# neobotix/neo_mpc_planner2

Hardware: AMD Instinct MI355X
Metric: MPC solves/sec (control_steps=3, 500x500 costmap) (higher is better)
Workload: dtype f64

## Files before the change

### neo_mpc_planner2_amd/csrc/costmap.h

```cpp
#pragma once
#include <hip/hip_runtime.h>
#include <math.h>
#include <stdint.h>

#include "neo_mpc_device.h"
#include "wave_ops.h"
#include "solver_context.h"
#include "fast_math.h"
#include "solver_rules.h"

namespace neo_mpc {
namespace {

__device__ __forceinline__ int cell_of(double w, double origin, double res, double inv) {
  double t = w - origin;
  double q = t * inv;
  double fl = floor(q);
  if (fabs(q - rint(q)) < 1e-6) fl = floor(t / res);
  int cell;
  asm("v_cvt_i32_f64 %0, %1" : "=v"(cell) : "v"(fl));
  return cell;
}

__device__ __forceinline__ int map_raw(const DevMap& m, int mx, int my) {
  if (mx < -m.border || my < -m.border || mx >= m.size_x + m.border || my >= m.size_y + m.border)
    return 254;
  return m.cells[(long)my * m.pitch + mx];
}

__device__ __forceinline__ int raw_occupancy(int raw) {
  return raw == 0 ? 0 : raw == 253 ? 99 : raw == 254 ? 100 : raw == 255 ? -1 : 1 + (97 * (raw - 1)) / 251;
}
__device__ __forceinline__ double raw_cost(int raw) { return (double)raw_occupancy(raw) / 100.0; }

template <bool kCovered = false>
__device__ __forceinline__ int cell_raw(const SolveArgs& a, const Ctx& c, const double* L, int mx, int my) {
  const unsigned tx = (unsigned)(mx - c.tile_x0), ty = (unsigned)(my - c.tile_y0);
  const int lg = c.tile_geom & 31;
  if (kCovered || ((tx >> lg) == 0u && ty < (unsigned)(c.tile_geom >> 8)))
    return reinterpret_cast<const uint8_t*>(L + a.lds.tile)[(ty << lg) + tx];
  return map_raw(a.map, mx, my);
}

template <bool kCovered = false>
__device__ __forceinline__ int step_raw(const SolveArgs& a, const Ctx& c, const double* L, double x, double y) {
  if (c.tile_geom & kTileFree) return 0;
  const double X = c.X0 + (c.c0 * x - c.s0 * y), Y = c.Y0 + (c.s0 * x + c.c0 * y);
  const int mx = cell_of(X, a.map.origin_x, a.map.resolution, a.map.inv_resolution);
  const int my = cell_of(Y, a.map.origin_y, a.map.resolution, a.map.inv_resolution);
  return cell_raw<kCovered>(a, c, L, mx, my);
}
template <bool kCovered = false>
__device__ __forceinline__ double step_term(const SolveArgs& a, const Ctx& c, const double* L, double x, double y) {
  return L[a.lds.term + step_raw<kCovered>(a, c, L, x, y)];
}

constexpr double kSticky = NEO_RULE_STICKY, kWall = NEO_RULE_WALL, kStickyDist = NEO_RULE_STICKY_DIST, kWallDist = NEO_RULE_WALL_DIST;
constexpr double kHopMargin = NEO_RULE_HOP_MARGIN;
template <bool kCovered = false>
__device__ __forceinline__ int edge_stickiness(const SolveArgs& a, const Ctx& c, const double* L, double x, double y,
                                               double cs, double sn, double& wxx, double& wxy, double& wyy, double& lx,
                                               double& ly, bool& hop, float& hop_x, float& hop_y) {
  wxx = 0.0; wxy = 0.0; wyy = 0.0; lx = 0.0; ly = 0.0;
  hop = false; hop_x = 0.0f; hop_y = 0.0f;
  if (c.tile_geom & kTileFree) return 0;
  const double X = c.X0 + (c.c0 * x - c.s0 * y), Y = c.Y0 + (c.s0 * x + c.c0 * y);
  const int mx = cell_of(X, a.map.origin_x, a.map.resolution, a.map.inv_resolution);
  const int my = cell_of(Y, a.map.origin_y, a.map.resolution, a.map.inv_resolution);
  const double fx = (X - a.map.origin_x) * a.map.inv_resolution - (double)mx;
  const double fy = (Y - a.map.origin_y) * a.map.inv_resolution - (double)my;
  const int raw_here = cell_raw<kCovered>(a, c, L, mx, my);
  const double here = L[a.lds.term + raw_here];
  const bool far = mx <= -2147483647 || mx >= 2147483646 || my <= -2147483647 || my >= 2147483646;
  if (far) return raw_here;
  const double hop_range = L[a.lds.tol + T_HOP_RANGE];
  const double zone = fmax(kWallDist, hop_range);
  const bool xlo = fx < zone, xhi = 1.0 - fx < zone, ylo = fy < zone, yhi = 1.0 - fy < zone;
  double rx = 0.0, ry = 0.0, pbx = 0.0, pby = 0.0;
  double drop = L[a.lds.tol + T_HOP_DROP], hwx = 0.0, hwy = 0.0;
  if (xlo || xhi) {
    const int raw_n = cell_raw<kCovered>(a, c, L, xlo ? mx - 1 : mx + 1, my);
    const double dist = xlo ? fx : 1.0 - fx, there = L[a.lds.term + raw_n];
    const bool wall = raw_n == 254 && raw_here != 254;
    if (wall) { if (dist < kWallDist) { rx = kWall * 2.0 * a.p.wt_n; pbx = (xlo ? kWallDist - dist : dist - kWallDist) * a.map.resolution; } }
    else if (dist < kStickyDist && there > here) rx = kSticky * 2.0 * a.p.wt_n;
    if (dist < hop_range && here - there > drop) {
      drop = here - there; hop = true;
      hwx = (xlo ? -1.0 : 1.0) * (dist + kHopMargin) * a.map.resolution; hwy = 0.0;
    }
  }
  if (ylo || yhi) {
    const int raw_n = cell_raw<kCovered>(a, c, L, mx, ylo ? my - 1 : my + 1);
    const double dist = ylo ? fy : 1.0 - fy, there = L[a.lds.term + raw_n];
    const bool wall = raw_n == 254 && raw_here != 254;
    if (wall) { if (dist < kWallDist) { ry = kWall * 2.0 * a.p.wt_n; pby = (ylo ? kWallDist - dist : dist - kWallDist) * a.map.resolution; } }
    else if (dist < kStickyDist && there > here) ry = kSticky * 2.0 * a.p.wt_n;
    if (dist < hop_range && here - there > drop) {
      hop = true;
      hwx = 0.0; hwy = (ylo ? -1.0 : 1.0) * (dist + kHopMargin) * a.map.resolution;
    }
  }
  wxx = rx * c.c0 * c.c0 + ry * c.s0 * c.s0;
  wxy = rx * c.c0 * -c.s0 + ry * c.s0 * c.c0;
  wyy = rx * c.s0 * c.s0 + ry * c.c0 * c.c0;
  lx = -(rx * pbx * c.c0 + ry * pby * c.s0);
  ly = -(rx * pbx * -c.s0 + ry * pby * c.c0);
  if (hop) {
    const double hrx = c.c0 * hwx + c.s0 * hwy, hry = -c.s0 * hwx + c.c0 * hwy, idt = rcp_fast(a.p.dt);
    hop_x = (float)((cs * hrx + sn * hry) * idt); hop_y = (float)((-sn * hrx + cs * hry) * idt);
  }
  return raw_here;
}

__device__ double edge_cost(const DevMap& m, double ax, double ay, double bx, double by) {
  int x0 = cell_of(ax, m.origin_x, m.resolution, m.inv_resolution);
  int y0 = cell_of(ay, m.origin_y, m.resolution, m.inv_resolution);
  const int x1 = cell_of(bx, m.origin_x, m.resolution, m.inv_resolution);
  const int y1 = cell_of(by, m.origin_y, m.resolution, m.inv_resolution);
  if (x0 < 0 || y0 < 0 || x0 >= m.size_x || y0 >= m.size_y || x1 < 0 || y1 < 0 || x1 >= m.size_x || y1 >= m.size_y)
    return raw_cost(254);
  const long dx = labs((long)x1 - x0), dy = labs((long)y1 - y0);
  const int sx = x1 >= x0 ? 1 : -1, sy = y1 >= y0 ? 1 : -1;
  long err = dx - dy;
  double worst = -1.0;
  for (long guard = 0; guard <= dx + dy + 1; ++guard) {
    worst = fmax(worst, raw_cost(map_raw(m, x0, y0)));
    if (x0 == x1 && y0 == y1) break;
    long e2 = 2 * err;
    if (e2 > -dy) { err -= dy; x0 += sx; }
    if (e2 < dx) { err += dx; y0 += sy; }
  }
  return worst;
}

__device__ double footprint_cost(const SolveArgs& a, const double* L, uint32_t b, int lane) {
  if (!a.footprints || a.footprint_points == 0) return L[a.lds.prob + P_FOOTPRINT];
  const int np = (int)a.footprint_points;
  const double* pts = a.footprints + (size_t)b * 2 * np;
  double worst = -1.0;
  for (int e = lane; e < np; e += kLanes) {
    int j = (e + 1) % np;
    worst = fmax(worst, edge_cost(a.map, pts[2 * e], pts[2 * e + 1], pts[2 * j], pts[2 * j + 1]));
  }
  return wave_max(worst);
}

}
}
```

### neo_mpc_planner2_amd/csrc/k1_solve.h

```cpp
#pragma once
#include <hip/hip_runtime.h>
#include <hip/hip_ext.h>
#include <math.h>
#include <stdint.h>
#include <stdlib.h>

#include "neo_mpc_device.h"
#include "wave_ops.h"
#include "fast_math.h"
#include "solver_context.h"
#include "solver_rules.h"
#include "costmap.h"
#include "feasible_set.h"
#include "rollout.h"
#include "riccati.h"
#include "adjoint.h"
#include "tangent_cone.h"
#include "dense_newton.h"
#include "lbfgs.h"
#include "cell_scan.h"
#include "k1_timing.h"

namespace neo_mpc {
namespace {
// ... 80 lines not shown
    load_records(a, L, b, lane);
    if (uniform_int(reinterpret_cast<const int*>(L + a.lds.prob)[PI_SKIP]) == 1) { skip_instance(a, b, lane); return false; }
    select_map(a.map, L + a.lds.prob);
    flags = reset_and_warm(a, L, b, lane) ? NEO_MPC_FLAG_RESET : 0;
    const double fcost = footprint_cost(a, L, b, lane);
    if (lane == 0) L[a.lds.prob + P_FOOTPRINT] = fcost;
    Ctx c;
    make_ctx_wave(p, a.map, L + a.lds.prob, fcost, c, lane);
    load_tile(a, c, L, lane);
    s.wall_in_reach = (c.tile_geom & kTileWall) != 0;
    if (s.wall_in_reach) flags |= NEO_MPC_FLAG_WALL_IN_REACH;
    if (lane == 0) {
      double* t = L + a.lds.tol;
      t[T_XTOL] = p.xtol; t[T_EARLY] = p.early_tol; t[T_FINAL] = p.final_tol; t[T_FTOL] = p.ftol;
      t[T_STALL] = p.stall_step; t[T_WTOL] = p.wtol; t[T_WTOL_LATE] = p.wtol_late; t[T_KINK] = p.kink_radius;
      t[T_KONST] = c.konst; t[T_TRUE_YAW] = c.true_yaw;
      t[T_HOP_DROP] = p.hop_min_drop; t[T_HOP_RANGE] = p.hop_range;
      t[T_BTOL_MAP] = p.btol_map; t[T_BTOL_FREE] = p.btol_free;
      reinterpret_cast<int*>(t + T_HOP_STAGE)[kHopLanes] = 0;
      t[T_C0] = c.c0; t[T_S0] = c.s0; t[T_TYAW] = c.tyaw; t[T_FYAW] = c.fyaw;
      int* ti = reinterpret_cast<int*>(t + T_TILE);
      ti[0] = c.tile_x0; ti[1] = c.tile_y0; ti[2] = c.tile_geom;
    }
    double* u = L + a.lds.u;
    for (int i = lane; i < n; i += kLanes) project_block<kTame>(p, u[3 * i], u[3 * i + 1], u[3 * i + 2]);
    WAVE_SYNC();
    for (int k = 0; k < nv; ++k) cold = cold && (u[k] == 0.0);
    ctx_from_lds<false>(a, L, c);
    {
      double* S = L + a.lds.state;
      int* Si = reinterpret_cast<int*>(S);
      const bool has_prev = uniform_int(Si[SI_HAS_PREV]) == 1 && !(flags & NEO_MPC_FLAG_RESET);
      WAVE_SYNC();
      if (lane == 0) {
        double q0 = has_prev ? S[S_PREV_U0] : u[nv - 3], q1 = has_prev ? S[S_PREV_U0 + 1] : u[nv - 2], q2 = has_prev ? S[S_PREV_U0 + 2] : u[nv - 1];
        project_block<kTame>(p, q0, q1, q2);
        S[S_PREV_U0] = q0; S[S_PREV_U0 + 1] = q1; S[S_PREV_U0 + 2] = q2;
        Si[SI_HAS_PREV] = 0;
      }
      WAVE_SYNC();
    }
    if (!cold && n > 1 && !(p.compat & kCompatNoUnshift) && p.max_it < kDumpGradient) {
      const double* A0 = L + a.lds.state + S_PREV_U0;
      double ts = 0.0;
      const double fs = rollout_cost<kSteps, kTame, kCovered>(
          a, c, L,
          [&](int i, double& b0, double& b1, double& b2) {
            const double* src = lane == 1 ? (i == 0 ? A0 : u + 3 * (i - 1)) : u + 3 * i;
            b0 = src[0]; b1 = src[1]; b2 = src[2];
          },
          NoRecord(), &ts);
      const double f_warm = lane_value(fs, 0), f_alt = lane_value(fs, 1);
      const bool free_both = lane_value(ts, 0) == 0.0 && lane_value(ts, 1) == 0.0;
      if (f_alt < f_warm && free_both) {
        double v0 = 0.0, v1 = 0.0, v2 = 0.0;
        const int k0 = lane, k1 = lane + kLanes, k2 = lane + 2 * kLanes;
        if (k0 < nv) v0 = k0 >= 3 ? u[k0 - 3] : A0[k0];
        if (k1 < nv) v1 = u[k1 - 3];
        if (k2 < nv) v2 = u[k2 - 3];
        WAVE_SYNC();
        if (k0 < nv) u[k0] = v0;
        if (k1 < nv) u[k1] = v1;
        if (k2 < nv) u[k2] = v2;
      } else if (f_alt < f_warm && lane == 0) {
        reinterpret_cast<int*>(L + a.lds.state)[SI_HAS_PREV] = kAltArmed;
      }
      WAVE_SYNC();
    }
  }
  s.flags = flags; s.cold = cold;
  return true;
}

template <int kMinWavesPerSimd, int kSteps, int kDir, bool kTame, int kStaticTile, int kLayoutSteps, bool kRouted = false>
__device__ __forceinline__ bool solve_search(double* L, uint32_t b, SolveCarry& sc) {
  constexpr bool kCovered = kStaticTile > 0;
  constexpr bool kNewton = kDir == 1;
  constexpr bool kRiccati = kDir == 2;
  constexpr bool kSecond = kDir != 0;
  constexpr bool kBlockedRule = kNewton || kRouted;
  static_assert(!kRiccati || kSteps == 0 || kRouted, "the stage-wise direction: run-time-sized, or the routed kernel's control_steps-3 branch");
  static_assert(!kRouted || (kRiccati && kSteps == kRoutedSteps), "the routed branch is the stage-wise one, three stages in registers");
  constexpr int kFew = (kRiccati && kSteps > 0) ? kSteps : 0;
  constexpr int kNwSteps = !kNewton ? 1 : kSteps ? kSteps : kNewtonMaxSteps;
  constexpr bool kVectorPose = kTame;
  constexpr int kRegSteps = kSteps ? kSteps : 1;
  constexpr int kPairs = kSteps ? 4 : NEO_MPC_MAX_LBFGS_MEMORY;
  double f = sc.f;
  const bool cold = sc.cold;
  int npairs = 0, head = 0, nfev = sc.nfev, it = sc.it, status = sc.status, stall = 0;
  int blocked_run = 0;
  int nblocked = 1;
  double u_term = 0.0;
  double gain1 = INFINITY, gain2 = INFINITY;
  bool final_step = false;
  double alpha = 1.0;
  bool scanned = false;
  int nscans = 0;
  bool scan_only = false;
  auto lane_again = []() {
    int zero;
    asm volatile("v_mov_b32 %0, 0" : "=v"(zero));
    return (int)__builtin_amdgcn_mbcnt_hi(~0u, __builtin_amdgcn_mbcnt_lo(~0u, (unsigned)zero));
  };
  NEO_SEGMENT_DECL;
  NEO_SEGMENT(0);
  for (;;) {
  SolveArgs a;
  fresh_args<kSteps, kStaticTile, kLayoutSteps, kRouted>(a);
  own_loop_params(a);
  select_map(a.map, L + a.lds.prob);
  const DevParams& p = a.p;
  const int n = kSteps ? kSteps : p.n, nv = 3 * n, mem = p.mem;
  double cand[3 * kRegSteps], cand_sn[kRegSteps], cand_cs[kRegSteps];
  bool have_trig = false;
  Ctx c;
  ctx_from_lds<kVectorPose>(a, L, c);
  double* u = L + a.lds.u;
  double* gs = L + a.lds.gs;
  double* gt = L + a.lds.gt;
  double* gr = L + a.lds.gr;
  double* d = L + a.lds.d;
  double* u_prev = L + a.lds.u_prev;
  double* gt_prev = L + a.lds.gt_prev;
  double* u_new = L + a.lds.u_new;
  double* ACS = L + a.lds.cs;
  double* ASN = L + a.lds.sn;
  int* AMODE = reinterpret_cast<int*>(L + a.lds.mode);
  static_assert(2 * 7 >= kNewtonRecord, "Newton records do not fit the step arrays");

  if (!scanned && nscans == 0) {
    const int lane = lane_again();
    for (int i = lane; i < n; i += kLanes) { AMODE[4 * i + 2] = 0; AMODE[4 * i + 3] = 0; }
    if (kRouted && lane == 0) L[a.lds.tol + T_KINK] = p.kink_radius_stagewise;
    alpha = kRiccati ? fmax(1.0, n * 0.125) : 1.0;
    if (kFew && lane == 0) { double* t = L + a.lds.tol; t[T_GAIN1] = INFINITY; t[T_GAIN2] = INFINITY; t[T_ALPHA] = alpha; }
    if (kRiccati && lane == 0) L[a.lds.tol + T_MU] = n > 8 ? (double)(n - 8) * 0.125 : 0.0;
  }
  bool v_feasible = false;
  if (kRiccati) {
    double b0 = c.v0, b1 = c.v1, b2 = c.v2;
    asm volatile("" : "+v"(b0), "+v"(b1), "+v"(b2));
    project_block<kTame>(p, b0, b1, b2);
    v_feasible = b0 == c.v0 && b1 == c.v1 && b2 == c.v2;
  }
  double my_scale;
  {
    int l0 = lane_again();
    my_scale = kRiccati ? 0.0 : lane_scale<kSecond>(l0);
  }
  for (; it < p.max_it && !scan_only; ++it) {
    int lane = lane_again();
    const bool exact_step = kRiccati && nblocked == 0;
    int tol_off = a.lds.tol;
    asm volatile("" : "+s"(tol_off));
    const double* TOL = L + tol_off;
    NEO_PHASE_DECL;
    NEO_PHASE(0);
    constexpr int kVars = 3 * kNwSteps;
    const int nvr = kSteps ? kVars : nv;
    bool free_path = false;
    int nhops = 0;
    float hc[kVars];
    float newton_sol = 0.0f;
    if (kNewton) {
      double hcol[kSteps ? kVars : 1];
      const double hstep = 1e-6, inv_h = 1.0 / hstep;
      double pcs[kNwSteps], psn[kNwSteps];
      double x = 0.0, y = 0.0, th = 0.0;
    #pragma unroll
      for (int i = 0; i < kNwSteps; ++i) {
        if (kSteps || i < n) {
          const double vx = u[3 * i] + (lane == 3 * i ? hstep : 0.0);
          const double vy = u[3 * i + 1] + (lane == 3 * i + 1 ? hstep : 0.0);
          const double w = u[3 * i + 2] + (lane == 3 * i + 2 ? hstep : 0.0);
          th += w * p.dt;
          sincos_heading<kTame>(th, &psn[i], &pcs[i]);
          x += (vx * pcs[i] - vy * psn[i]) * p.dt;
          y += (vx * psn[i] + vy * pcs[i]) * p.dt;
        }
      }
      double SX = 0.0, SY = 0.0, ST = 0.0;
    #pragma unroll
      for (int k = kNwSteps - 1; k >= 0; --k) {
        if (kSteps || k < n) {
          const double vx = u[3 * k] + (lane == 3 * k ? hstep : 0.0);
          const double vy = u[3 * k + 1] + (lane == 3 * k + 1 ? hstep : 0.0);
          const double w = u[3 * k + 2] + (lane == 3 * k + 2 ? hstep : 0.0);
          const double pdx = (vx * pcs[k] - vy * psn[k]) * p.dt, pdy = (vx * psn[k] + vy * pcs[k]) * p.dt;
          double prt = -2.0 * p.wo_n * (c.tyaw - th);
          if (k == n - 1) prt += -2.0 * p.wterm_o * (c.fyaw - th);
          SX += -2.0 * p.wt_n * (c.cx - x); SY += -2.0 * p.wt_n * (c.cy - y);
          ST += prt - pdy * SX + pdx * SY;
          const double g0 = p.dt * (pcs[k] * SX + psn[k] * SY), g1 = p.dt * (-psn[k] * SX + pcs[k] * SY),
                       g2 = p.dt * ST;
          if (kSteps) {
            hcol[3 * k] = g0; hcol[3 * k + 1] = g1; hcol[3 * k + 2] = g2;
          } else {
            const double b0 = lane_value(g0, 63), b1 = lane_value(g1, 63), b2 = lane_value(g2, 63);
            if (lane == 63) { gs[3 * k] = b0; gs[3 * k + 1] = b1; gs[3 * k + 2] = b2; }
            hc[3 * k] = (float)((g0 - b0) * inv_h);
            hc[3 * k + 1] = (float)((g1 - b1) * inv_h);
            hc[3 * k + 2] = (float)((g2 - b2) * inv_h);
          }
          x -= pdx; y -= pdy; th -= w * p.dt;
        } else {
          hc[3 * k] = 0.0f; hc[3 * k + 1] = 0.0f; hc[3 * k + 2] = 0.0f;
        }
      }
      if (kSteps) {
    #pragma unroll
        for (int j = 0; j < kVars; ++j) {
          const double base = lane_value(hcol[j], 63);
          if (lane == 63) gs[j] = base;
          hc[j] = (float)((hcol[j] - base) * inv_h);
        }
      }
      WAVE_SYNC();
    }
    else if (!kSteps || kRiccati) adjoint_by_scans<kTame, kRiccati, kFew>(a, c, L, exact_step, lane, n, free_path, nhops);
    else adjoint_short_sweep<kSteps, kTame>(a, c, L, have_trig, lane, n);
    NEO_PHASE(1);
    const bool my_corner = tangent_cone_pass<kTame, kNewton, kRiccati>(a, c, L, TOL[T_KINK], lane, n);
    WAVE_SYNC();
    const bool corner_any = kSecond && !kTame && __ballot(my_corner) != 0ull && (kRiccati ? free_path : (it > 0 && u_term == 0.0));
    NEO_PHASE(2);
    if (p.max_it == kDumpGradient) {
      for (int k = lane; k < nv; k += kLanes) a.solution[(size_t)b * nv + k] = gt[k];
      return true;
    }
    if (kSecond && it == 0 && cold) {
      if (kRiccati) { for (int k = lane; k < nv; k += kLanes) d[k] = -gr[k]; }
      else if (lane < nvr) d[lane] = -gr[lane];
      if (kRiccati) for (int i = lane; i < n; i += kLanes) AMODE[4 * i + 3] = 0;
      WAVE_SYNC();
    } else if (kRiccati) {
      riccati_prepare(a, c, L, n, lane, v_feasible, (float)TOL[T_MU]);
      WAVE_SYNC();
      if (corner_any) riccati_keep_linear_terms(a, L, n, lane, true);
      auto sweep = [&]() {
        riccati_sweep<float, (kMinWavesPerSimd < 4), kFew>(a, L, n, lane);
        riccati_finish(a, c, L, n, lane);
      };
      sweep();
      if (!kTame && corner_any && repin_corner_blocks<true>(a, L, n, lane)) {
        riccati_keep_linear_terms(a, L, n, lane, false);
        sweep();
      }
    } else if (kNewton) {
      newton_sol = dense_newton_direction<kSteps, kNwSteps, kTame>(a, L, hc, corner_any, lane, n, nvr);
    }
    NEO_PHASE(3);
    if (!kSecond) lbfgs_direction<kSteps, kPairs>(a, L, it, mem, head, npairs, lane, n);
    if (kSecond && it > 0) {
      float dm = 0.0f;
      int anynear = 0;
      if (kRiccati) {
        for (int k = lane; k < nv; k += kLanes) {
          const float v = (float)fabs(d[k]);
          dm = (v == v) ? fmaxf(dm, v) : INFINITY;
          anynear |= (AMODE[4 * (k / 3) + 2] == 1);
        }
      } else if (lane < nvr) { dm = fabsf(newton_sol); anynear = (AMODE[4 * (lane / 3) + 2] == 1); }
      if constexpr (kFew > 0 && 3 * kFew <= 16) dm = wave_max_f_few<3 * kFew>(dm); else dm = wave_max_f(dm);
      const bool near_any = __ballot(anynear != 0) != 0ull;
      if ((double)dm < TOL[T_EARLY] && !near_any && nhops == 0) { status = NEO_MPC_STATUS_CONVERGED; break; }
      if ((double)dm < ((kRiccati && !exact_step) ? kFinalFracGaussNewton : 1.0) * TOL[T_FINAL] && !near_any) final_step = true;
    }
    NEO_PHASE(4);
    if (p.max_it > kDumpGradient && it == p.max_it - kDumpGradient - 1) {
      for (int k = lane; k < nv; k += kLanes) a.solution[(size_t)b * nv + k] = d[k];
      return true;
    }
    const double lscale = kRiccati ? lane_scale<kSecond>(lane) : my_scale;
    const double alpha_now = kFew ? TOL[T_ALPHA] : alpha;
    const double pstep = alpha_now * lscale;
    const double step = lane < 32 ? pstep : lscale;
    bool took_trial = false;
    double fb = INFINITY, cterm = 0.0;
    int best = 32;
    if (kRiccati && free_path && it > 0) took_trial = riccati_free_space_trial<kTame, kCovered, kFew, kBlockedRule>(a, c, L, n, lane, alpha_now, f, fb, cterm);
    const double* ALT0 = L + a.lds.state + S_PREV_U0;
    bool alt_armed = false;
    if (it == 0) alt_armed = uniform_int(reinterpret_cast<const int*>(L + a.lds.state)[SI_HAS_PREV]) == kAltArmed;
    if (!took_trial) {
    int hop_stage = -1;
    float hop_x = 0.0f, hop_y = 0.0f;
    if (kRiccati && lane >= 1 && lane <= nhops) {
      const double* t = TOL;
      hop_stage = reinterpret_cast<const int*>(t + T_HOP_STAGE)[lane - 1];
      hop_x = reinterpret_cast<const float*>(t + T_HOP_VEC)[2 * (lane - 1)];
      hop_y = reinterpret_cast<const float*>(t + T_HOP_VEC)[2 * (lane - 1) + 1];
    }
    double fc = rollout_cost<kSteps, kTame, kCovered>(
        a, c, L,
        [&](int i, double& b0, double& b1, double& b2) {
          candidate_block<kTame, kRiccati, (kFew > 0 && kTame)>(a, c, L, lane, step, pstep, i, b0, b1, b2, hop_stage, hop_x, hop_y);
          if (it == 0) {
            asm volatile("");
            if (lane == 0) { b0 = u[3 * i]; b1 = u[3 * i + 1]; b2 = u[3 * i + 2]; }
            if (lane == kAltLane && alt_armed) { const double* src = i == 0 ? ALT0 : u + 3 * (i - 1); b0 = src[0]; b1 = src[1]; b2 = src[2]; }
          }
          if (kSteps) { cand[3 * i] = b0; cand[3 * i + 1] = b1; cand[3 * i + 2] = b2; }
        },
        [&](int i, double sn, double cs) {
          if (kSteps && !kSecond) { cand_sn[i] = sn; cand_cs[i] = cs; }
        }, kBlockedRule ? &cterm : nullptr);
    NEO_PHASE(5);
    if (!(fc == fc)) fc = INFINITY;
    if (it == 0) { f = lane_value(fc, 0); if (kNewton) u_term = lane_value(cterm, 0); }
    fb = fc;
    best = lane;
    wave_argmin(fb, best);
    }
    ++nfev;
    if (!(fb < f)) { status = NEO_MPC_STATUS_CONVERGED; ++it; break; }
    const bool alt_won = alt_armed && best == kAltLane;
    float stepmax = 0.0f;
    if (kSteps && kSecond && !took_trial) {
      if (lane == best) {
#pragma unroll
        for (int k = 0; k < 3 * kRegSteps; ++k) {
          stepmax = fmaxf(stepmax, (float)fabs(cand[k] - u[k]));
          u[k] = cand[k];
        }
      }
      stepmax = __builtin_bit_cast(float, __builtin_amdgcn_readlane(__builtin_bit_cast(int, stepmax), best));
      have_trig = true;
    } else {
      if (kSteps && !kSecond) {
        if (lane == best) {
#pragma unroll
          for (int i = 0; i < kRegSteps; ++i) {
            u_new[3 * i] = cand[3 * i]; u_new[3 * i + 1] = cand[3 * i + 1]; u_new[3 * i + 2] = cand[3 * i + 2];
            ASN[i] = cand_sn[i]; ACS[i] = cand_cs[i];
          }
        }
      } else if (!kSteps && !took_trial) {
        const double bstep = lane_value(step, best), bpstep = lane_value(pstep, best);
        int bhop = -1;
        float bhx = 0.0f, bhy = 0.0f;
        if (kRiccati && best >= 1 && best <= nhops) {
          bhop = reinterpret_cast<const int*>(TOL + T_HOP_STAGE)[best - 1];
          bhx = reinterpret_cast<const float*>(TOL + T_HOP_VEC)[2 * (best - 1)];
          bhy = reinterpret_cast<const float*>(TOL + T_HOP_VEC)[2 * (best - 1) + 1];
        }
        for (int i = lane; i < n; i += kLanes) {
// ... 187 lines not shown
```

### neo_mpc_planner2_amd/csrc/riccati.h

```cpp
#pragma once
#include <hip/hip_runtime.h>
#include <math.h>
#include <stdint.h>

#include "neo_mpc_device.h"
#include "wave_ops.h"
#include "fast_math.h"
#include "solver_context.h"
#include "solver_rules.h"
#include "costmap.h"
#include "feasible_set.h"

namespace neo_mpc {
namespace {

enum : int {
  RS_PX = 0, RS_PY, RS_TX, RS_TY,
  RS_WXX, RS_WXY, RS_WYY, RS_FLAGS,
  RS_C00, RS_C01, RS_C02, RS_C11,
  RS_C12, RS_C22, RS_CS, RS_SN,
  RS_GT = 16,
  RS_GS = 19,
  RS_WK = 22,
  RS_WLX = 25, RS_WLY,
  RS_SY = 27,
  RS_GAIN = 16,
  kRicStage = 28
};
enum : int { RC_FREE3 = 0, RC_SLIDE_W, RC_XY, RC_SLIDE, RC_W, RC_NONE, RC_KINK, RF_CASE = 7, RF_KINK_OK = 8 };

typedef float ric_f4 __attribute__((ext_vector_type(4)));

__device__ __forceinline__ float ric_rcp(float x) { return __builtin_amdgcn_rcpf(x); }
__device__ __forceinline__ double ric_rcp(double x) { return rcp_fast(x); }
template <typename T> __device__ __forceinline__ T ric_max(T a, T b) { return a > b ? a : b; }
template <typename T> __device__ __forceinline__ T ric_abs(T a) { return a < (T)0 ? -a : a; }
__device__ __forceinline__ float ric_fma(float a, float b, float c) { return fmaf(a, b, c); }
__device__ __forceinline__ double ric_fma(double a, double b, double c) { return fma(a, b, c); }
template <typename T> __device__ __forceinline__ T ric_pivot(T p, T delta) { return p > delta ? p : ric_max(ric_abs(p), delta); }
__device__ __forceinline__ float ric_floor(float a) { return fmaxf(a, 1e-30f); }
__device__ __forceinline__ double ric_floor(double a) { return ric_max(a, 1e-30); }
__device__ __forceinline__ float ric_mag(float a) { return fabsf(a); }
__device__ __forceinline__ double ric_mag(double a) { return ric_abs(a); }
__device__ __forceinline__ float ric_pivot(float p, float delta) { return fmaxf(fabsf(p), delta); }

__device__ __forceinline__ void riccati_prepare(const SolveArgs& a, const Ctx& c, double* L, int n, int lane,
                                                bool v_feasible, float mu) {
  if (lane >= n) return;
  const DevParams& p = a.p;
  float* rs = reinterpret_cast<float*>(L + a.lds.ric) + kRicStage * lane;
  const int* am = reinterpret_cast<const int*>(L + a.lds.mode) + 4 * lane;
  const double* gt = L + a.lds.gt + 3 * lane;
  const double* gs = L + a.lds.gs + 3 * lane;
  const double* u = L + a.lds.u + 3 * lane;
  const double cs = rs[RS_CS], sn = rs[RS_SN];
  const double idt = rcp_fast(p.dt);
  rs[RS_GT] = (float)((cs * gt[0] - sn * gt[1]) * idt); rs[RS_GT + 1] = (float)((sn * gt[0] + cs * gt[1]) * idt);
  rs[RS_GT + 2] = (float)(gt[2] * idt);
  rs[RS_GS] = (float)((cs * gs[0] - sn * gs[1]) * idt); rs[RS_GS + 1] = (float)((sn * gs[0] + cs * gs[1]) * idt);
  rs[RS_GS + 2] = (float)(gs[2] * idt);
  const double e0 = u[0] - c.v0, e1 = u[1] - c.v1, e2 = u[2] - c.v2;
  rs[RS_WK] = (float)(-(cs * e0 - sn * e1) * p.dt); rs[RS_WK + 1] = (float)(-(sn * e0 + cs * e1) * p.dt);
  rs[RS_WK + 2] = (float)(-e2 * p.dt);
  const double nx = L[a.lds.nx + lane], ny = L[a.lds.ny + lane];
  const double tx = -ny, ty = nx;
  const float rtx = (float)(cs * tx - sn * ty), rty = (float)(sn * tx + cs * ty);
  rs[RS_TX] = rtx; rs[RS_TY] = rty;
  const int near = am[2];
  const int xy = near ? 2 : am[0];
  const bool wfree = !(near || (am[1] & 1));
  const int kase = xy == 0 ? (wfree ? RC_FREE3 : RC_XY) : xy == 1 ? (wfree ? RC_SLIDE_W : RC_SLIDE) : (wfree ? RC_W : RC_NONE);
  const int flags = kase | ((!near && v_feasible) ? RF_KINK_OK : 0);
  rs[RS_FLAGS] = (float)flags;
  float c00 = 0.0f, c01 = 0.0f, c02 = 0.0f, c11 = 0.0f, c12 = 0.0f, c22 = 0.0f;
  if (!near) {
    const float f0 = (float)(cs * e0 - sn * e1), f1 = (float)(sn * e0 + cs * e1), f2 = (float)e2;
    const float fn2 = f0 * f0 + f1 * f1 + f2 * f2;
    const float ine = fn2 > 0.0f ? __builtin_amdgcn_rsqf(fn2) : 0.0f;
    const float i2 = (float)(idt * idt);
    const float sN = (float)p.wc_n * ine * i2, h0 = f0 * ine, h1 = f1 * ine, h2 = f2 * ine;
    const float k2 = reinterpret_cast<const float*>(L + a.lds.rt)[2 * lane] * i2;
    c00 = sN * (1.0f - h0 * h0) + k2 * rtx * rtx; c01 = -sN * h0 * h1 + k2 * rtx * rty; c02 = -sN * h0 * h2;
    c11 = sN * (1.0f - h1 * h1) + k2 * rty * rty; c12 = -sN * h1 * h2; c22 = sN * (1.0f - h2 * h2);
    const float mt = mu * (float)(2.0 * p.wt_n);
    c00 += mt; c11 += mt; c22 += mu * (float)(2.0 * p.wo_n);
  }
  rs[RS_C00] = c00; rs[RS_C01] = c01; rs[RS_C02] = c02; rs[RS_C11] = c11; rs[RS_C12] = c12; rs[RS_C22] = c22;
}

__device__ __forceinline__ void riccati_keep_linear_terms(const SolveArgs& a, double* L, int n, int lane, bool save) {
  ric_f4* rec = reinterpret_cast<ric_f4*>(reinterpret_cast<float*>(L + a.lds.ric) + kRicStage * lane + RS_GAIN);
  ric_f4* keep = reinterpret_cast<ric_f4*>(L + a.lds.keep) + 3 * lane;
  for (int i = lane; i < n; i += kLanes, rec += 7 * kLanes, keep += 3 * kLanes) {
    if (save) { keep[0] = rec[0]; keep[1] = rec[1]; keep[2] = rec[2]; }
    else { rec[0] = keep[0]; rec[1] = keep[1]; rec[2] = keep[2]; }
  }
  WAVE_SYNC();
}

template <typename T, bool kPrefetch = true, int kFew = 0>
__device__ __forceinline__ void riccati_sweep(const SolveArgs& a, double* L, int n, int lane) {
  const DevParams& p = a.p;
  float* RS = static_cast<float*>(__builtin_assume_aligned(reinterpret_cast<float*>(L + a.lds.ric), 16));
  int* AMODE = reinterpret_cast<int*>(L + a.lds.mode);
  double* d = L + a.lds.d;
  const float* ARTF = reinterpret_cast<const float*>(L + a.lds.rt);
  const T w2 = (T)(2.0 * p.wt_n), wo2 = (T)(2.0 * p.wo_n), wterm2 = (T)(2.0 * p.wterm_o);
  const T wc2 = (T)((p.wc_n * p.wc_n) / (p.dt * p.dt));

  T V00 = (T)0.0, V01 = (T)0.0, V02 = (T)0.0, V11 = (T)0.0, V12 = (T)0.0, V22 = (T)0.0, v0 = (T)0.0, v1 = (T)0.0, v2 = (T)0.0;
  ric_f4 r0, r1, r2, r3, r4, r5, r6;
  if (kPrefetch) {
    const ric_f4* R4 = reinterpret_cast<const ric_f4*>(RS + kRicStage * (n - 1));
    r0 = R4[0]; r1 = R4[1]; r2 = R4[2]; r3 = R4[3]; r4 = R4[4]; r5 = R4[5]; r6 = R4[6];
  }
  for (int i = (kFew ? kFew : n) - 1; i >= 0; --i) {
    const bool first = kFew > 0 && i == 0;
    if (!kPrefetch) {
      const ric_f4* R4 = reinterpret_cast<const ric_f4*>(RS + kRicStage * i);
      r0 = R4[0]; r1 = R4[1]; r2 = R4[2]; r3 = R4[3]; r4 = R4[4]; r5 = R4[5]; r6 = R4[6];
    }
    const T px = r0.x, py = r0.y, rtx = r0.z, rty = r0.w;
    const T wxx = r1.x, wxy = r1.y, wyy = r1.z;
    const int flags = __builtin_amdgcn_readfirstlane((int)r1.w);
    const T c00 = r2.x, c01 = r2.y, c02 = r2.z, c11 = r2.w, c12 = r3.x, c22 = r3.y;
    const T gt0 = r4.x, gt1 = r4.y, gt2 = r4.z, gs0 = r4.w, gs1 = r5.x, gs2 = r5.y, e0 = r5.z, e1 = r5.w, e2 = r6.x;
    v0 += (T)r6.y; v1 += (T)r6.z;
    const T sy = (T)r6.w, sx = (T)ARTF[2 * i + 1];
    if (kPrefetch && i > 0) {
      const ric_f4* R4 = reinterpret_cast<const ric_f4*>(RS + kRicStage * (i - 1));
      r0 = R4[0]; r1 = R4[1]; r2 = R4[2]; r3 = R4[3]; r4 = R4[4]; r5 = R4[5]; r6 = R4[6];
    }
    const T S00 = V00 + w2 + wxx, S01 = V01 + wxy, S11 = V11 + w2 + wyy;
    const T S22 = V22 + wo2 + (i == n - 1 ? wterm2 : (T)0.0);
    const T M02 = ric_fma(-py, S00, ric_fma(px, S01, V02));
    const T M12 = ric_fma(-py, S01, ric_fma(px, S11, V12));
    const T M22 = ric_fma(-py, M02, ric_fma(px, M12, ric_fma(-py, V02, ric_fma(px, V12, S22))));
    const T Z02 = M02 + sy, Z12 = M12 - sx, Z22 = M22 - ric_fma(sx, px, sy * py);
    const T z0 = v0, z1 = v1, z2 = ric_fma(-py, v0, ric_fma(px, v1, v2));
    T k0 = (T)0.0, k1 = (T)0.0, k2 = (T)0.0, K00 = (T)0.0, K01 = (T)0.0, K02 = (T)0.0, K10 = (T)0.0, K11 = (T)0.0, K12 = (T)0.0,
      K20 = (T)0.0, K21 = (T)0.0, K22 = (T)0.0;
    bool tokink = false;
    int kase = flags & RF_CASE;
    if (flags & RF_KINK_OK) {
      const T q0 = gs0 + z0 + S00 * e0 + S01 * e1 + Z02 * e2;
      const T q1 = gs1 + z1 + S01 * e0 + S11 * e1 + Z12 * e2;
      const T q2 = gs2 + z2 + Z02 * e0 + Z12 * e1 + Z22 * e2;
      if (__builtin_amdgcn_readfirstlane((int)(q0 * q0 + q1 * q1 + q2 * q2 <= wc2))) { tokink = true; kase = RC_KINK; }
    }
    const T q0 = gt0 + z0, q1 = gt1 + z1, q2 = gt2 + z2;
    switch (kase) {
      case RC_FREE3: {
        const T Q00 = S00 + c00, Q01 = S01 + c01, Q02 = Z02 + c02, Q11 = S11 + c11, Q12 = Z12 + c12, Q22 = Z22 + c22;
        const T delta = ric_floor((T)1e-6 * ric_max(ric_mag(Q00), ric_max(ric_mag(Q11), ric_mag(Q22))));
        const T d0 = ric_pivot(Q00, delta), i0 = ric_rcp(d0);
        const T l10 = Q01 * i0, l20 = Q02 * i0;
        const T d1 = ric_pivot(Q11 - l10 * Q01, delta), i1 = ric_rcp(d1);
        const T h12 = Q12 - l20 * Q01;
        const T l21 = h12 * i1;
        const T d2 = ric_pivot(Q22 - l20 * Q02 - l21 * h12, delta), i2 = ric_rcp(d2);
#define NEO_RIC_SOLVE3(r0_, r1_, r2_, x0_, x1_, x2_)                                           \
        {                                                                                        \
          const T y0 = -(r0_), y1 = -(r1_) - l10 * y0, y2 = -(r2_) - l20 * y0 - l21 * y1;        \
          x2_ = y2 * i2;                                                                         \
          x1_ = y1 * i1 - l21 * x2_;                                                             \
          x0_ = y0 * i0 - l10 * x1_ - l20 * x2_;                                                 \
        }
        NEO_RIC_SOLVE3(q0, q1, q2, k0, k1, k2)
        if (first) break;
        NEO_RIC_SOLVE3(S00, S01, M02, K00, K10, K20)
        NEO_RIC_SOLVE3(S01, S11, M12, K01, K11, K21)
        NEO_RIC_SOLVE3(Z02, Z12, Z22, K02, K12, K22)
#undef NEO_RIC_SOLVE3
        v0 = z0 + S00 * k0 + S01 * k1 + M02 * k2;
        v1 = z1 + S01 * k0 + S11 * k1 + M12 * k2;
        v2 = z2 + Z02 * k0 + Z12 * k1 + Z22 * k2;
        V00 = S00 + S00 * K00 + S01 * K10 + M02 * K20;
        V01 = S01 + S00 * K01 + S01 * K11 + M02 * K21;
        V02 = M02 + S00 * K02 + S01 * K12 + M02 * K22;
        V11 = S11 + S01 * K01 + S11 * K11 + M12 * K21;
        V12 = M12 + S01 * K02 + S11 * K12 + M12 * K22;
        V22 = Z22 + Z02 * K02 + Z12 * K12 + Z22 * K22;
        break;
      }
      case RC_SLIDE_W:
      case RC_XY: {
        const bool bw = kase == RC_SLIDE_W;
        const T ax = bw ? rtx : (T)1.0, ay = bw ? rty : (T)0.0;
        const T Q00 = S00 + c00, Q01 = S01 + c01, Q11 = S11 + c11;
        const T Qa0 = ax * Q00 + ay * Q01, Qa1 = ax * Q01 + ay * Q11;
        const T haa = Qa0 * ax + Qa1 * ay;
        const T hab = bw ? ax * (Z02 + c02) + ay * (Z12 + c12) : Qa1;
        const T hbb = bw ? Z22 + c22 : Q11;
        const T ga = ax * q0 + ay * q1, gb = bw ? q2 : q1;
        const T Za0 = ax * S00 + ay * S01, Za1 = ax * S01 + ay * S11, Za2 = ax * Z02 + ay * Z12;
        const T Zb0 = bw ? M02 : S01, Zb1 = bw ? M12 : S11, Zb2 = bw ? Z22 : Z12;
        const T delta = ric_floor((T)1e-6 * ric_max(ric_mag(haa), ric_mag(hbb)));
        const T d0 = ric_pivot(haa, delta), i0 = ric_rcp(d0);
        const T l = hab * i0;
        const T d1 = ric_pivot(hbb - l * hab, delta), i1 = ric_rcp(d1);
        T ka, kb, Ka0, Ka1, Ka2, Kb0, Kb1, Kb2;
#define NEO_RIC_SOLVE2(ra_, rb_, xa_, xb_)                       \
        {                                                          \
          const T y0 = -(ra_), y1 = -(rb_) - l * y0;               \
          xb_ = y1 * i1;                                           \
          xa_ = y0 * i0 - l * xb_;                                 \
        }
        NEO_RIC_SOLVE2(ga, gb, ka, kb)
        if (first) {
          k0 = ax * ka; k1 = ay * ka;
          if (bw) k2 = kb; else k1 = kb;
          break;
        }
        NEO_RIC_SOLVE2(Za0, Zb0, Ka0, Kb0)
        NEO_RIC_SOLVE2(Za1, Zb1, Ka1, Kb1)
        NEO_RIC_SOLVE2(Za2, Zb2, Ka2, Kb2)
#undef NEO_RIC_SOLVE2
        v0 = z0 + Za0 * ka + Zb0 * kb; v1 = z1 + Za1 * ka + Zb1 * kb; v2 = z2 + Za2 * ka + Zb2 * kb;
        V00 = S00 + Za0 * Ka0 + Zb0 * Kb0; V01 = S01 + Za0 * Ka1 + Zb0 * Kb1; V02 = M02 + Za0 * Ka2 + Zb0 * Kb2;
        V11 = S11 + Za1 * Ka1 + Zb1 * Kb1; V12 = M12 + Za1 * Ka2 + Zb1 * Kb2; V22 = Z22 + Za2 * Ka2 + Zb2 * Kb2;
        k0 = ax * ka; k1 = ay * ka; K00 = ax * Ka0; K01 = ax * Ka1; K02 = ax * Ka2; K10 = ay * Ka0; K11 = ay * Ka1; K12 = ay * Ka2;
        if (bw) { k2 = kb; K20 = Kb0; K21 = Kb1; K22 = Kb2; }
        else { k1 = kb; K10 = Kb0; K11 = Kb1; K12 = Kb2; }
        break;
      }
      case RC_SLIDE: {
        const T Q00 = S00 + c00, Q01 = S01 + c01, Q11 = S11 + c11;
        const T haa = (rtx * Q00 + rty * Q01) * rtx + (rtx * Q01 + rty * Q11) * rty;
        const T i0 = -ric_rcp(ric_pivot(haa, ric_floor((T)1e-6 * ric_mag(haa))));
        const T Za0 = rtx * S00 + rty * S01, Za1 = rtx * S01 + rty * S11, Za2 = rtx * Z02 + rty * Z12;
        const T ka = (rtx * q0 + rty * q1) * i0, Ka0 = Za0 * i0, Ka1 = Za1 * i0, Ka2 = Za2 * i0;
        if (first) { k0 = rtx * ka; k1 = rty * ka; break; }
        v0 = z0 + Za0 * ka; v1 = z1 + Za1 * ka; v2 = z2 + Za2 * ka;
        V00 = S00 + Za0 * Ka0; V01 = S01 + Za0 * Ka1; V02 = M02 + Za0 * Ka2;
        V11 = S11 + Za1 * Ka1; V12 = M12 + Za1 * Ka2; V22 = Z22 + Za2 * Ka2;
        k0 = rtx * ka; k1 = rty * ka; K00 = rtx * Ka0; K01 = rtx * Ka1; K02 = rtx * Ka2; K10 = rty * Ka0; K11 = rty * Ka1; K12 = rty * Ka2;
        break;
      }
      case RC_W: {
        const T hbb = Z22 + c22;
        const T i0 = -ric_rcp(ric_pivot(hbb, ric_floor((T)1e-6 * ric_mag(hbb))));
        k2 = q2 * i0;
        if (first) break;
        K20 = M02 * i0; K21 = M12 * i0; K22 = Z22 * i0;
        v0 = z0 + M02 * k2; v1 = z1 + M12 * k2; v2 = z2 + Z22 * k2;
        V00 = S00 + M02 * K20; V01 = S01 + M02 * K21; V02 = M02 + M02 * K22;
        V11 = S11 + M12 * K21; V12 = M12 + M12 * K22; V22 = Z22 + Z22 * K22;
        break;
      }
      case RC_KINK:
        k0 = e0; k1 = e1; k2 = e2;
        if (first) break;
        v0 = z0 + S00 * k0 + S01 * k1 + M02 * k2;
        v1 = z1 + S01 * k0 + S11 * k1 + M12 * k2;
        v2 = z2 + Z02 * k0 + Z12 * k1 + Z22 * k2;
        V00 = S00; V01 = S01; V02 = M02; V11 = S11; V12 = M12; V22 = Z22;
        break;
      default:
        v0 = z0; v1 = z1; v2 = z2;
        V00 = S00; V01 = S01; V02 = M02; V11 = S11; V12 = M12; V22 = Z22;
        break;
    }
    if (lane == 0) {
      ric_f4* G4 = reinterpret_cast<ric_f4*>(RS + kRicStage * i + RS_GAIN);
      G4[0] = ric_f4{(float)K00, (float)K01, (float)K02, (float)K10};
      G4[1] = ric_f4{(float)K11, (float)K12, (float)K20, (float)K21};
      G4[2] = ric_f4{(float)K22, (float)k0, (float)k1, (float)k2};
      AMODE[4 * i + 3] = tokink ? 1 : 0;
    }
  }
  WAVE_SYNC();
  T z0 = (T)0.0, z1 = (T)0.0, z2 = (T)0.0;
  ric_f4 fs[kFew ? kFew : 1][4];
  if (kFew) {
    for (int i = 0; i < kFew; ++i) {
      const ric_f4* R4 = reinterpret_cast<const ric_f4*>(RS + kRicStage * i);
      fs[i][0] = R4[0]; fs[i][1] = R4[4]; fs[i][2] = R4[5]; fs[i][3] = R4[6];
    }
  }
  for (int i = 0; i < (kFew ? kFew : n); ++i) {
    const ric_f4* R4 = reinterpret_cast<const ric_f4*>(RS + kRicStage * i);
    const ric_f4 s0 = kFew ? fs[i][0] : R4[0], g0 = kFew ? fs[i][1] : R4[4], g1 = kFew ? fs[i][2] : R4[5], g2 = kFew ? fs[i][3] : R4[6];
    const T w0 = (T)g2.y + (T)g0.x * z0 + (T)g0.y * z1 + (T)g0.z * z2;
    const T w1 = (T)g2.z + (T)g0.w * z0 + (T)g1.x * z1 + (T)g1.y * z2;
    const T w2f = (T)g2.w + (T)g1.z * z0 + (T)g1.w * z1 + (T)g2.x * z2;
    if (lane == 0) { d[3 * i] = (double)w0; d[3 * i + 1] = (double)w1; d[3 * i + 2] = (double)w2f; }
    const T e0 = z0 + w0, e1 = z1 + w1, e2 = z2 + w2f;
    z0 = ric_fma(-(T)s0.y, e2, e0); z1 = ric_fma((T)s0.x, e2, e1); z2 = e2;
  }
  WAVE_SYNC();
}

__device__ __forceinline__ void riccati_finish(const SolveArgs& a, const Ctx& c, double* L, int n, int lane) {
  if (lane < n) {
    const float* rs = reinterpret_cast<const float*>(L + a.lds.ric) + kRicStage * lane;
    const int* am = reinterpret_cast<const int*>(L + a.lds.mode) + 4 * lane;
    double* d = L + a.lds.d + 3 * lane;
    if (am[3]) {
      const double* u = L + a.lds.u + 3 * lane;
      d[0] = c.v0 - u[0]; d[1] = c.v1 - u[1]; d[2] = c.v2 - u[2];
    } else {
      const double cs = rs[RS_CS], sn = rs[RS_SN], idt = rcp_fast(a.p.dt);
      const double w0 = d[0], w1 = d[1], w2 = d[2];
      double d0 = (cs * w0 + sn * w1) * idt, d1 = (-sn * w0 + cs * w1) * idt;
      const int mode = am[2] ? 2 : am[0];
      if (mode == 1) {
        const double nx = L[a.lds.nx + lane], ny = L[a.lds.ny + lane];
        const double dot = d0 * nx + d1 * ny;
        d0 -= dot * nx; d1 -= dot * ny;
      } else if (mode == 2) { d0 = 0.0; d1 = 0.0; }
      d[0] = d0; d[1] = d1; d[2] = (am[2] || (am[1] & 1)) ? 0.0 : w2 * idt;
    }
  }
  WAVE_SYNC();
}

template <bool kTame, bool kCovered, int kFew, bool kWantTerm>
__device__ __forceinline__ bool riccati_free_space_trial(const SolveArgs& a, const Ctx& c, double* L, int n, int lane,
                                                         double alpha_now, double f, double& fb, double& cterm) {
  constexpr double kTrialRatio = NEO_RULE_TRIAL_RATIO;
  const DevParams& p = a.p;
  const double *u = L + a.lds.u, *gr = L + a.lds.gr;
  double* u_new = L + a.lds.u_new;
  bool took_trial = false;
  const bool on = lane < n;
  double b0 = 0.0, b1 = 0.0, b2 = 0.0, g0 = 0.0, g1 = 0.0, g2 = 0.0;
  if (on) {
    candidate_block<kTame, true>(a, c, L, 32, 1.0, alpha_now, lane, b0, b1, b2);
    g0 = gr[3 * lane]; g1 = gr[3 * lane + 1]; g2 = gr[3 * lane + 2];
    u_new[3 * lane] = b0; u_new[3 * lane + 1] = b1; u_new[3 * lane + 2] = b2;
  }
  auto scan = [](double v) { if constexpr (kFew > 0) return wave_scan_few<kFew>(v); else return wave_scan(v); };
  auto sum = [](double v) { if constexpr (kFew > 0) return wave_sum_few<kFew>(v); else return wave_sum(v); };
  const double th = scan(b2 * p.dt);
  double sn, cs;
  sincos_heading<kTame>(th, &sn, &cs);
  const double x = scan((b0 * cs - b1 * sn) * p.dt), y = scan((b0 * sn + b1 * cs) * p.dt);
  double fi = 0.0, pr = 0.0, tm = 0.0;
  if (on) {
    const double dx = c.cx - x, dy = c.cy - y, et = c.tyaw - th;
    const double e0 = c.v0 - b0, e1 = c.v1 - b1, e2 = c.v2 - b2;
    tm = step_term<kCovered>(a, c, L, x, y);
    fi = p.wt_n * (dx * dx + dy * dy) + p.wo_n * (et * et) + p.wc_n * sqrt_fast(e0 * e0 + e1 * e1 + e2 * e2) + tm;
    if (lane == n - 1) { const double ef = c.fyaw - th; fi += p.wterm_o * (ef * ef); }
    pr = -0.5 * (g0 * (b0 - u[3 * lane]) + g1 * (b1 - u[3 * lane + 1]) + g2 * (b2 - u[3 * lane + 2]));
  }
  const double ft = sum(fi), pred = sum(pr);
  if (ft < f && f - ft >= kTrialRatio * pred) {
    took_trial = true; fb = ft;
    if (kWantTerm) cterm = sum(tm);
  }
  WAVE_SYNC();
  return took_trial;
}

}
}
```

Before: 25.79 million.

## Hand off Riccati sweep results to finish step in registers instead of LDS

For the fixed-step (control_steps=3) Riccati path, the sweep now passes per-stage feedforward values, modes, controls and rotation terms to the finish step through a register struct. This removes one wave sync and the LDS round trip between the two phases. The finish step also computes each lane's step-magnitude max directly, so the convergence check can skip rereading d and AMODE from LDS. Stage flags are broadcast with readlane so the sweep treats them as scalars, and wt_n is pinned to an SGPR in edge_stickiness. The cost is more register pressure and extra code paths that must stay consistent with the LDS-based path.

```diff
diff --git a/neo_mpc_planner2_amd/csrc/costmap.h b/neo_mpc_planner2_amd/csrc/costmap.h
--- a/neo_mpc_planner2_amd/csrc/costmap.h
+++ b/neo_mpc_planner2_amd/csrc/costmap.h
@@ -64,6 +64,8 @@
   wxx = 0.0; wxy = 0.0; wyy = 0.0; lx = 0.0; ly = 0.0;
   hop = false; hop_x = 0.0f; hop_y = 0.0f;
   if (c.tile_geom & kTileFree) return 0;
+  double wt_n = a.p.wt_n;
+  asm volatile("" : "+s"(wt_n));
   const double X = c.X0 + (c.c0 * x - c.s0 * y), Y = c.Y0 + (c.s0 * x + c.c0 * y);
   const int mx = cell_of(X, a.map.origin_x, a.map.resolution, a.map.inv_resolution);
   const int my = cell_of(Y, a.map.origin_y, a.map.resolution, a.map.inv_resolution);
@@ -82,8 +84,8 @@
     const int raw_n = cell_raw<kCovered>(a, c, L, xlo ? mx - 1 : mx + 1, my);
     const double dist = xlo ? fx : 1.0 - fx, there = L[a.lds.term + raw_n];
     const bool wall = raw_n == 254 && raw_here != 254;
-    if (wall) { if (dist < kWallDist) { rx = kWall * 2.0 * a.p.wt_n; pbx = (xlo ? kWallDist - dist : dist - kWallDist) * a.map.resolution; } }
-    else if (dist < kStickyDist && there > here) rx = kSticky * 2.0 * a.p.wt_n;
+    if (wall) { if (dist < kWallDist) { rx = kWall * 2.0 * wt_n; pbx = (xlo ? kWallDist - dist : dist - kWallDist) * a.map.resolution; } }
+    else if (dist < kStickyDist && there > here) rx = kSticky * 2.0 * wt_n;
     if (dist < hop_range && here - there > drop) {
       drop = here - there; hop = true;
       hwx = (xlo ? -1.0 : 1.0) * (dist + kHopMargin) * a.map.resolution; hwy = 0.0;
@@ -93,8 +95,8 @@
     const int raw_n = cell_raw<kCovered>(a, c, L, mx, ylo ? my - 1 : my + 1);
     const double dist = ylo ? fy : 1.0 - fy, there = L[a.lds.term + raw_n];
     const bool wall = raw_n == 254 && raw_here != 254;
-    if (wall) { if (dist < kWallDist) { ry = kWall * 2.0 * a.p.wt_n; pby = (ylo ? kWallDist - dist : dist - kWallDist) * a.map.resolution; } }
-    else if (dist < kStickyDist && there > here) ry = kSticky * 2.0 * a.p.wt_n;
+    if (wall) { if (dist < kWallDist) { ry = kWall * 2.0 * wt_n; pby = (ylo ? kWallDist - dist : dist - kWallDist) * a.map.resolution; } }
+    else if (dist < kStickyDist && there > here) ry = kSticky * 2.0 * wt_n;
     if (dist < hop_range && here - there > drop) {
       hop = true;
       hwx = 0.0; hwy = (ylo ? -1.0 : 1.0) * (dist + kHopMargin) * a.map.resolution;
diff --git a/neo_mpc_planner2_amd/csrc/k1_solve.h b/neo_mpc_planner2_amd/csrc/k1_solve.h
--- a/neo_mpc_planner2_amd/csrc/k1_solve.h
+++ b/neo_mpc_planner2_amd/csrc/k1_solve.h
@@ -186,6 +186,8 @@
   static_assert(!kRiccati || kSteps == 0 || kRouted, "the stage-wise direction: run-time-sized, or the routed kernel's control_steps-3 branch");
   static_assert(!kRouted || (kRiccati && kSteps == kRoutedSteps), "the routed branch is the stage-wise one, three stages in registers");
   constexpr int kFew = (kRiccati && kSteps > 0) ? kSteps : 0;
+  constexpr bool kHandOff = kFew > 0;
+  constexpr bool kScalarCase = kFew > 0 && kTame;
   constexpr int kNwSteps = !kNewton ? 1 : kSteps ? kSteps : kNewtonMaxSteps;
   constexpr bool kVectorPose = kTame;
   constexpr int kRegSteps = kSteps ? kSteps : 1;
@@ -267,6 +269,8 @@
     int nhops = 0;
     float hc[kVars];
     float newton_sol = 0.0f;
+    float dm_reg = 0.0f;
+    int near_reg = 0;
     if (kNewton) {
       double hcol[kSteps ? kVars : 1];
       const double hstep = 1e-6, inv_h = 1.0 / hstep;
@@ -339,12 +343,18 @@
       if (kRiccati) for (int i = lane; i < n; i += kLanes) AMODE[4 * i + 3] = 0;
       WAVE_SYNC();
     } else if (kRiccati) {
-      riccati_prepare(a, c, L, n, lane, v_feasible, (float)TOL[T_MU]);
+      const int my_flags = riccati_prepare(a, c, L, n, lane, v_feasible, (float)TOL[T_MU]);
+      int stage_flags[kFew ? kFew : 1] = {};
+      if (kScalarCase) {
+        for (int i = 0; i < kFew; ++i) stage_flags[i] = __builtin_amdgcn_readlane(my_flags, i);
+      }
       WAVE_SYNC();
       if (corner_any) riccati_keep_linear_terms(a, L, n, lane, true);
       auto sweep = [&]() {
-        riccati_sweep<float, (kMinWavesPerSimd < 4), kFew>(a, L, n, lane);
-        riccati_finish(a, c, L, n, lane);
+        SweepHandOff<float> ho = {};
+        riccati_sweep<float, (kMinWavesPerSimd < 4), kFew, kHandOff, kScalarCase>(a, L, n, lane, &ho, stage_flags);
+        riccati_finish<kHandOff>(a, c, L, n, lane, &ho, &dm_reg);
+        near_reg = ho.near;
       };
       sweep();
       if (!kTame && corner_any && repin_corner_blocks<true>(a, L, n, lane)) {
@@ -359,14 +369,18 @@
     if (kSecond && it > 0) {
       float dm = 0.0f;
       int anynear = 0;
-      if (kRiccati) {
+      if (kHandOff) {
+        dm = dm_reg;
+        anynear = near_reg == 1;
+      } else if (kRiccati) {
         for (int k = lane; k < nv; k += kLanes) {
           const float v = (float)fabs(d[k]);
           dm = (v == v) ? fmaxf(dm, v) : INFINITY;
           anynear |= (AMODE[4 * (k / 3) + 2] == 1);
         }
       } else if (lane < nvr) { dm = fabsf(newton_sol); anynear = (AMODE[4 * (lane / 3) + 2] == 1); }
-      if constexpr (kFew > 0 && 3 * kFew <= 16) dm = wave_max_f_few<3 * kFew>(dm); else dm = wave_max_f(dm);
+      if constexpr (kHandOff) dm = wave_max_f_few<kFew>(dm);
+      else if constexpr (kFew > 0 && 3 * kFew <= 16) dm = wave_max_f_few<3 * kFew>(dm); else dm = wave_max_f(dm);
       const bool near_any = __ballot(anynear != 0) != 0ull;
       if ((double)dm < TOL[T_EARLY] && !near_any && nhops == 0) { status = NEO_MPC_STATUS_CONVERGED; break; }
       if ((double)dm < ((kRiccati && !exact_step) ? kFinalFracGaussNewton : 1.0) * TOL[T_FINAL] && !near_any) final_step = true;
diff --git a/neo_mpc_planner2_amd/csrc/riccati.h b/neo_mpc_planner2_amd/csrc/riccati.h
--- a/neo_mpc_planner2_amd/csrc/riccati.h
+++ b/neo_mpc_planner2_amd/csrc/riccati.h
@@ -44,9 +44,9 @@
 __device__ __forceinline__ double ric_mag(double a) { return ric_abs(a); }
 __device__ __forceinline__ float ric_pivot(float p, float delta) { return fmaxf(fabsf(p), delta); }
 
-__device__ __forceinline__ void riccati_prepare(const SolveArgs& a, const Ctx& c, double* L, int n, int lane,
-                                                bool v_feasible, float mu) {
-  if (lane >= n) return;
+__device__ __forceinline__ int riccati_prepare(const SolveArgs& a, const Ctx& c, double* L, int n, int lane,
+                                               bool v_feasible, float mu) {
+  if (lane >= n) return 0;
   const DevParams& p = a.p;
   float* rs = reinterpret_cast<float*>(L + a.lds.ric) + kRicStage * lane;
   const int* am = reinterpret_cast<const int*>(L + a.lds.mode) + 4 * lane;
@@ -86,6 +86,7 @@
     c00 += mt; c11 += mt; c22 += mu * (float)(2.0 * p.wo_n);
   }
   rs[RS_C00] = c00; rs[RS_C01] = c01; rs[RS_C02] = c02; rs[RS_C11] = c11; rs[RS_C12] = c12; rs[RS_C22] = c22;
+  return flags;
 }
 
 __device__ __forceinline__ void riccati_keep_linear_terms(const SolveArgs& a, double* L, int n, int lane, bool save) {
@@ -98,8 +99,18 @@
   WAVE_SYNC();
 }
 
-template <typename T, bool kPrefetch = true, int kFew = 0>
-__device__ __forceinline__ void riccati_sweep(const SolveArgs& a, double* L, int n, int lane) {
+template <typename T>
+struct SweepHandOff {
+  T w0, w1, w2;
+  unsigned tokink;
+  double u0, u1, u2, nx, ny;
+  float cs, sn;
+  int mode, wfroz, near;
+};
+template <typename T, bool kPrefetch = true, int kFew = 0, bool kHandOff = false, bool kScalarCase = false>
+__device__ __forceinline__ void riccati_sweep(const SolveArgs& a, double* L, int n, int lane, SweepHandOff<T>* ho = nullptr,
+                                              const int* stage_flags = nullptr) {
+  static_assert(!(kHandOff || kScalarCase) || kFew > 0, "register hand-offs: the unrolled sweeps");
   const DevParams& p = a.p;
   float* RS = static_cast<float*>(__builtin_assume_aligned(reinterpret_cast<float*>(L + a.lds.ric), 16));
   int* AMODE = reinterpret_cast<int*>(L + a.lds.mode);
@@ -122,7 +133,7 @@
     }
     const T px = r0.x, py = r0.y, rtx = r0.z, rty = r0.w;
     const T wxx = r1.x, wxy = r1.y, wyy = r1.z;
-    const int flags = __builtin_amdgcn_readfirstlane((int)r1.w);
+    const int flags = kScalarCase ? stage_flags[kFew ? i : 0] : __builtin_amdgcn_readfirstlane((int)r1.w);
     const T c00 = r2.x, c01 = r2.y, c02 = r2.z, c11 = r2.w, c12 = r3.x, c22 = r3.y;
     const T gt0 = r4.x, gt1 = r4.y, gt2 = r4.z, gs0 = r4.w, gs1 = r5.x, gs2 = r5.y, e0 = r5.z, e1 = r5.w, e2 = r6.x;
     v0 += (T)r6.y; v1 += (T)r6.z;
@@ -268,6 +279,7 @@
       G4[2] = ric_f4{(float)K22, (float)k0, (float)k1, (float)k2};
       AMODE[4 * i + 3] = tokink ? 1 : 0;
     }
+    if (kHandOff && tokink) ho->tokink |= 1u << i;
   }
   WAVE_SYNC();
   T z0 = (T)0.0, z1 = (T)0.0, z2 = (T)0.0;
@@ -277,6 +289,14 @@
       const ric_f4* R4 = reinterpret_cast<const ric_f4*>(RS + kRicStage * i);
       fs[i][0] = R4[0]; fs[i][1] = R4[4]; fs[i][2] = R4[5]; fs[i][3] = R4[6];
     }
+    if (kHandOff && lane < kFew) {
+      const int* am = AMODE + 4 * lane;
+      const double* u = L + a.lds.u + 3 * lane;
+      ho->mode = am[0]; ho->wfroz = am[1]; ho->near = am[2];
+      ho->u0 = u[0]; ho->u1 = u[1]; ho->u2 = u[2];
+      ho->nx = L[a.lds.nx + lane]; ho->ny = L[a.lds.ny + lane];
+      ho->cs = RS[kRicStage * lane + RS_CS]; ho->sn = RS[kRicStage * lane + RS_SN];
+    }
   }
   for (int i = 0; i < (kFew ? kFew : n); ++i) {
     const ric_f4* R4 = reinterpret_cast<const ric_f4*>(RS + kRicStage * i);
@@ -284,33 +304,62 @@
     const T w0 = (T)g2.y + (T)g0.x * z0 + (T)g0.y * z1 + (T)g0.z * z2;
     const T w1 = (T)g2.z + (T)g0.w * z0 + (T)g1.x * z1 + (T)g1.y * z2;
     const T w2f = (T)g2.w + (T)g1.z * z0 + (T)g1.w * z1 + (T)g2.x * z2;
-    if (lane == 0) { d[3 * i] = (double)w0; d[3 * i + 1] = (double)w1; d[3 * i + 2] = (double)w2f; }
+    if (kHandOff) { if (lane == i) { ho->w0 = w0; ho->w1 = w1; ho->w2 = w2f; } }
+    else if (lane == 0) { d[3 * i] = (double)w0; d[3 * i + 1] = (double)w1; d[3 * i + 2] = (double)w2f; }
     const T e0 = z0 + w0, e1 = z1 + w1, e2 = z2 + w2f;
     z0 = ric_fma(-(T)s0.y, e2, e0); z1 = ric_fma((T)s0.x, e2, e1); z2 = e2;
   }
-  WAVE_SYNC();
-}
-
-__device__ __forceinline__ void riccati_finish(const SolveArgs& a, const Ctx& c, double* L, int n, int lane) {
+  if (!kHandOff) WAVE_SYNC();
+}
+
+template <bool kHandOff = false, typename T = float>
+__device__ __forceinline__ void riccati_finish(const SolveArgs& a, const Ctx& c, double* L, int n, int lane,
+                                               const SweepHandOff<T>* ho = nullptr, float* dmax = nullptr) {
+  double dr[3] = {0.0, 0.0, 0.0};
   if (lane < n) {
     const float* rs = reinterpret_cast<const float*>(L + a.lds.ric) + kRicStage * lane;
-    const int* am = reinterpret_cast<const int*>(L + a.lds.mode) + 4 * lane;
     double* d = L + a.lds.d + 3 * lane;
+    int am[4];
+    double u[3] = {0.0, 0.0, 0.0}, nx = 0.0, ny = 0.0;
+    float fcs = 0.0f, fsn = 0.0f;
+    T hw0 = (T)0.0, hw1 = (T)0.0, hw2 = (T)0.0;
+    if (kHandOff) {
+      am[0] = ho->mode; am[1] = ho->wfroz; am[2] = ho->near; am[3] = (int)((ho->tokink >> lane) & 1u);
+      u[0] = ho->u0; u[1] = ho->u1; u[2] = ho->u2; nx = ho->nx; ny = ho->ny; fcs = ho->cs; fsn = ho->sn;
+      hw0 = ho->w0; hw1 = ho->w1; hw2 = ho->w2;
+      asm("" : "+v"(hw0), "+v"(hw1), "+v"(hw2));
+    } else {
+      const int* amL = reinterpret_cast<const int*>(L + a.lds.mode) + 4 * lane;
+      am[0] = amL[0]; am[1] = amL[1]; am[2] = amL[2]; am[3] = amL[3];
+    }
     if (am[3]) {
-      const double* u = L + a.lds.u + 3 * lane;
-      d[0] = c.v0 - u[0]; d[1] = c.v1 - u[1]; d[2] = c.v2 - u[2];
+      if (!kHandOff) { const double* uL = L + a.lds.u + 3 * lane; u[0] = uL[0]; u[1] = uL[1]; u[2] = uL[2]; }
+      const double k0 = c.v0 - u[0], k1 = c.v1 - u[1], k2 = c.v2 - u[2];
+      d[0] = k0; d[1] = k1; d[2] = k2;
+      if (kHandOff) { dr[0] = k0; dr[1] = k1; dr[2] = k2; }
     } else {
-      const double cs = rs[RS_CS], sn = rs[RS_SN], idt = rcp_fast(a.p.dt);
-      const double w0 = d[0], w1 = d[1], w2 = d[2];
+      const double cs = kHandOff ? fcs : rs[RS_CS], sn = kHandOff ? fsn : rs[RS_SN], idt = rcp_fast(a.p.dt);
+      const double w0 = kHandOff ? (double)hw0 : d[0], w1 = kHandOff ? (double)hw1 : d[1], w2 = kHandOff ? (double)hw2 : d[2];
       double d0 = (cs * w0 + sn * w1) * idt, d1 = (-sn * w0 + cs * w1) * idt;
       const int mode = am[2] ? 2 : am[0];
       if (mode == 1) {
-        const double nx = L[a.lds.nx + lane], ny = L[a.lds.ny + lane];
+        if (!kHandOff) { nx = L[a.lds.nx + lane]; ny = L[a.lds.ny + lane]; }
         const double dot = d0 * nx + d1 * ny;
         d0 -= dot * nx; d1 -= dot * ny;
       } else if (mode == 2) { d0 = 0.0; d1 = 0.0; }
-      d[0] = d0; d[1] = d1; d[2] = (am[2] || (am[1] & 1)) ? 0.0 : w2 * idt;
-    }
+      const double d2 = (am[2] || (am[1] & 1)) ? 0.0 : w2 * idt;
+      d[0] = d0; d[1] = d1; d[2] = d2;
+      if (kHandOff) { dr[0] = d0; dr[1] = d1; dr[2] = d2; }
+    }
+  }
+  if (kHandOff) {
+    float dm = 0.0f;
+#pragma unroll
+    for (int j = 0; j < 3; ++j) {
+      const float v = (float)fabs(dr[j]);
+      dm = (v == v) ? fmaxf(dm, v) : INFINITY;
+    }
+    *dmax = dm;
   }
   WAVE_SYNC();
 }
```

Result: faster. 26.88 million, median of 6 (+4.2%).
